# SobeyMIL/MVOC

Hardware: AMD Instinct MI355X
Metric: UNet3D denoising steps/sec, 16x512^2 frames, inversion+compose (higher is better)
Workload: dtype f16

## Files before the change

include/mvoc_hip.h:

```cpp
#ifndef MVOC_HIP_H
#define MVOC_HIP_H

#include <stddef.h>
#include <stdint.h>

#ifdef __cplusplus
extern "C" {
#endif

#define MVOC_VERSION 100

int mvoc_version(void);
const char* mvoc_last_error(void);

enum { MVOC_A_PLAIN = 0, MVOC_A_CONV3X3 = 1, MVOC_A_TEMPORAL3 = 2 };
enum { MVOC_ACT_NONE = 0, MVOC_ACT_GEGLU = 1, MVOC_ACT_SILU = 2, MVOC_ACT_GELU = 3 };

typedef struct mvoc_gemm_desc {
  const void* a;
  const void* a2;
  const void* w;
  void* out;
  const void* bias;
  const void* rowadd;
  const void* resid;
  int64_t m, n, k;
  int32_t n_store;
  int32_t ldo, ldr, ld_rowadd, rowadd_div;
  int32_t a_mode;
  int32_t lda, lda2;
  int32_t c1;
  int32_t cin;
  int32_t nimg, hout, wout, hsrc, wsrc, stride, upsample, hup, wup;
  int32_t frames, hw;
  int32_t act;
  int32_t tile;
  int32_t split_k;
  void* workspace;
  size_t workspace_bytes;
  const void* ln_rowsum;
  const void* ln_bias;
  float ln_eps;
  int32_t pad_mode;
  const void* ln_stats;
  void* chan_sums;
  void* row_moments;
// ... 196 lines not shown
```

mvoc_amd/_ffi.py:

```python
import ctypes as C
import os

import torch

_HERE = os.path.dirname(os.path.abspath(__file__))
LIB_PATH = os.environ.get("MVOC_HIP_LIB") or os.path.join(_HERE, "libmvoc_hip.so")

ABI_VERSION = 100

A_PLAIN, A_CONV3X3, A_TEMPORAL3 = 0, 1, 2
ACT_NONE, ACT_GEGLU, ACT_SILU, ACT_GELU = 0, 1, 2, 3
FAMILIES = ("gemm", "flash_attn", "temporal_attn", "groupnorm", "layernorm", "pnp", "misc", "temporal_fused")

vp, i32, i64, f32, f64, sz = C.c_void_p, C.c_int32, C.c_int64, C.c_float, C.c_double, C.c_size_t


class GemmDesc(C.Structure):
    _fields_ = [("a", vp), ("a2", vp), ("w", vp), ("out", vp), ("bias", vp), ("rowadd", vp), ("resid", vp),
                ("m", i64), ("n", i64), ("k", i64), ("n_store", i32), ("ldo", i32), ("ldr", i32), ("ld_rowadd", i32),
                ("rowadd_div", i32), ("a_mode", i32), ("lda", i32), ("lda2", i32), ("c1", i32), ("cin", i32),
                ("nimg", i32), ("hout", i32), ("wout", i32), ("hsrc", i32), ("wsrc", i32), ("stride", i32),
                ("upsample", i32), ("hup", i32), ("wup", i32), ("frames", i32), ("hw", i32), ("act", i32), ("tile", i32),
                ("split_k", i32), ("workspace", vp), ("workspace_bytes", sz), ("ln_rowsum", vp), ("ln_bias", vp),
                ("ln_eps", f32), ("pad_mode", i32), ("ln_stats", vp), ("chan_sums", vp), ("row_moments", vp),
# ... 11 lines not shown
class TAttnDesc(C.Structure):
    _fields_ = [("q", vp), ("k", vp), ("v", vp), ("out", vp),
                ("q_bs", i64), ("q_ps", i64), ("q_ts", i64), ("k_bs", i64), ("k_ps", i64), ("k_ts", i64),
                ("v_bs", i64), ("v_ps", i64), ("v_ts", i64), ("o_bs", i64), ("o_ps", i64), ("o_ts", i64),
                ("nsample", i32), ("hw", i32), ("heads", i32), ("frames", i32)]


class GnDesc(C.Structure):
    _fields_ = [("x", vp), ("x2", vp), ("gamma", vp), ("beta", vp), ("out", vp), ("workspace", vp),
                ("workspace_bytes", sz), ("nsample", i32), ("rows_per_sample", i32), ("c", i32), ("c1", i32),
                ("groups", i32), ("silu", i32), ("eps", f32), ("chan_sums", vp), ("chan_sums2", vp)]


class TFusedDesc(C.Structure):
    _fields_ = [("x", vp), ("wp", vp), ("ln_rowsum", vp), ("ln_bias", vp), ("out", vp), ("nsample", i32), ("frames", i32),
                ("hw", i32), ("c", i32), ("heads", i32), ("ln_eps", f32)]


class XsDesc(C.Structure):
    _fields_ = [("x", vp), ("wp", vp), ("resid", vp), ("out", vp), ("m", i64),
                ("n", i32), ("k", i32), ("n_store", i32), ("ldo", i32), ("ldr", i32), ("act", i32), ("normalize", i32),
                ("ln_eps", C.c_float), ("wp_set_rows", i64)]


class PnpDesc(C.Structure):
    _fields_ = [("x", vp), ("x2", vp), ("masks", vp), ("chunk_stride", i64), ("f_stride", i64), ("p_stride", i64),
                ("nobj", i32), ("frames", i32), ("height", i32), ("width", i32), ("channels", i32), ("mask_h", i32),
                ("mask_w", i32), ("base_chunk0", i32), ("ndst", i32)]


SIGNATURES = {
    "mvoc_version": (i32, []),
    "mvoc_last_error": (C.c_char_p, []),
    "mvoc_gemm_f16": (i32, [C.POINTER(GemmDesc), vp]),
    "mvoc_gemm_workspace_bytes": (sz, [i64, i64, i64]),
    "mvoc_gemm_chan_sums_written": (i32, []),
    "mvoc_gemm_row_moments_written": (i32, []),
    "mvoc_row_stats_from_moments_f32": (i32, [vp, i64, i32, i32, i32, f32, vp, vp]),
    "mvoc_flash_attn_f16": (i32, [C.POINTER(AttnDesc), vp]),
    "mvoc_temporal_attn_f16": (i32, [C.POINTER(TAttnDesc), vp]),
    "mvoc_temporal_qkv_attn_f16": (i32, [C.POINTER(TFusedDesc), vp]),
    "mvoc_xs_linear_f16": (i32, [C.POINTER(XsDesc), vp]),
    "mvoc_groupnorm_workspace_bytes": (sz, [i32, i32, i32, i32]),
    "mvoc_groupnorm_f16": (i32, [C.POINTER(GnDesc), vp]),
    "mvoc_groupnorm_fold_xs_f16": (i32, [C.POINTER(GnDesc), vp, vp, i32, i32, vp, vp]),
    "mvoc_groupnorm_moments_f16": (i32, [C.POINTER(GnDesc), vp, vp]),
    "mvoc_groupnorm_apply_moments_f16": (i32, [C.POINTER(GnDesc), vp, i32, vp]),
    "mvoc_layernorm_f16": (i32, [vp, vp, vp, vp, i64, i32, f32, vp]),
    "mvoc_row_stats_f16": (i32, [vp, vp, i64, i32, f32, vp]),
    "mvoc_pnp_blend_scatter_tokens": (i32, [C.POINTER(PnpDesc), vp]),
    "mvoc_pnp_blend_scatter_nchw": (i32, [C.POINTER(PnpDesc), vp]),
    "mvoc_pnp_blend_scatter_tokens_mapped": (i32, [C.POINTER(PnpDesc), i32, C.POINTER(i32), vp]),
    "mvoc_pnp_blend_scatter_nchw_mapped": (i32, [C.POINTER(PnpDesc), i32, C.POINTER(i32), vp]),
    "mvoc_pnp_blend_scatter_tokens_variants": (i32, [C.POINTER(PnpDesc), i32, C.POINTER(i32), i32, vp]),
    "mvoc_pnp_blend_scatter_nchw_variants": (i32, [C.POINTER(PnpDesc), i32, C.POINTER(i32), i32, vp]),
    "mvoc_pnp_blend_scatter_tokens_variants_sel": (i32, [C.POINTER(PnpDesc), i32, C.POINTER(i32), i32, C.c_uint32, vp]),
    "mvoc_pnp_blend_scatter_nchw_variants_sel": (i32, [C.POINTER(PnpDesc), i32, C.POINTER(i32), i32, C.c_uint32, vp]),
    "mvoc_pnp_blend_scatter_tokens_placed": (i32, [C.POINTER(PnpDesc), i32, C.POINTER(i32), i32, C.c_uint32, vp, vp]),
    "mvoc_pnp_blend_scatter_nchw_placed": (i32, [C.POINTER(PnpDesc), i32, C.POINTER(i32), i32, C.c_uint32, vp, vp]),
    "mvoc_pnp_blend_scatter_tokens_placed_variants": (i32, [C.POINTER(PnpDesc), i32, C.POINTER(i32), i32, C.c_uint32, vp, vp]),
    "mvoc_pnp_blend_scatter_nchw_placed_variants": (i32, [C.POINTER(PnpDesc), i32, C.POINTER(i32), i32, C.c_uint32, vp, vp]),
    "mvoc_shift_planes_f16": (i32, [vp, vp, i32, i32, i32, i32, vp, vp]),
    "mvoc_pnp_blend_scatter_tokens_resampled": (i32, [C.POINTER(PnpDesc), i32, C.POINTER(i32), i32, C.c_uint32, vp, vp]),
    "mvoc_pnp_blend_scatter_nchw_resampled": (i32, [C.POINTER(PnpDesc), i32, C.POINTER(i32), i32, C.c_uint32, vp, vp]),
    "mvoc_pnp_blend_scatter_tokens_resampled_variants": (i32, [C.POINTER(PnpDesc), i32, C.POINTER(i32), i32, C.c_uint32, vp, vp]),
    "mvoc_pnp_blend_scatter_nchw_resampled_variants": (i32, [C.POINTER(PnpDesc), i32, C.POINTER(i32), i32, C.c_uint32, vp, vp]),
# ... 71 lines not shown
```

mvoc_amd/csrc/runtime.hip:

```cpp
#include <stdarg.h>

#include <mutex>
#include <vector>

#include "common.h"

namespace {
thread_local char g_err[512] = "";

struct ProfRec {
  hipEvent_t e0, e1;
  int fam;
  double work;
};
std::mutex g_prof_mu;
bool g_prof_on = false;
std::vector<ProfRec*> g_prof_recs;
}

void mvoc_set_error(const char* fmt, ...) {
  va_list ap;
  va_start(ap, fmt);
  vsnprintf(g_err, sizeof(g_err), fmt, ap);
  va_end(ap);
}

int mvoc_check_launch(const char* what) {
  hipError_t e = hipGetLastError();
  if (e != hipSuccess) {
    mvoc_set_error("%s: %s", what, hipGetErrorString(e));
    return -3;
  }
  return 0;
}

MvocProfScope::MvocProfScope(int fam_, hipStream_t s, double work) : fam(fam_), stream(s), rec(nullptr) {
  if (!g_prof_on) return;
  ProfRec* r = new ProfRec;
  r->fam = fam_;
  r->work = work;
  if (hipEventCreate(&r->e0) != hipSuccess || hipEventCreate(&r->e1) != hipSuccess) {
    delete r;
    return;
  }
  (void)hipEventRecord(r->e0, s);
  rec = r;
}

MvocProfScope::~MvocProfScope() {
  if (!rec) return;
  ProfRec* r = (ProfRec*)rec;
  (void)hipEventRecord(r->e1, stream);
  std::lock_guard<std::mutex> lk(g_prof_mu);
  g_prof_recs.push_back(r);
}

extern "C" int mvoc_version(void) { return MVOC_VERSION; }
extern "C" const char* mvoc_last_error(void) { return g_err; }

extern "C" int mvoc_prof_enable(int on) {
  g_prof_on = on != 0;
  return 0;
}

extern "C" int mvoc_prof_reset(void) {
  std::lock_guard<std::mutex> lk(g_prof_mu);
  for (ProfRec* r : g_prof_recs) {
    (void)hipEventDestroy(r->e0);
    (void)hipEventDestroy(r->e1);
    delete r;
  }
  g_prof_recs.clear();
  return 0;
}

extern "C" int mvoc_prof_collect(double* ms, int64_t* launches, double* work) {
  std::lock_guard<std::mutex> lk(g_prof_mu);
  for (int i = 0; i < MVOC_FAM_COUNT; ++i) {
    if (ms) ms[i] = 0;
    if (launches) launches[i] = 0;
    if (work) work[i] = 0;
  }
  for (ProfRec* r : g_prof_recs) {
    float t = 0;
    if (hipEventElapsedTime(&t, r->e0, r->e1) != hipSuccess) {
      mvoc_set_error("prof_collect: event not complete (synchronise the stream first)");
      return -3;
    }
    if (ms) ms[r->fam] += t;
// ... 6 lines not shown
```

mvoc_amd/csrc/xslin.hip:

```cpp
#include <stdlib.h>

#include "common.h"

namespace {

struct XsArgs {
  const half_t* x;
  const half_t* wp;
  const half_t* resid;
  half_t* out;
  long M;
  int N, n_store, ldo, ldr, act, normalize;
  float eps;
  unsigned long long* stamps;
  int lab;
  long set_rows;
  long set_bytes;
};

#ifdef MVOC_PP_LAB
#define XS_STAMP(t) asm volatile("s_memtime %0\n\ts_waitcnt lgkmcnt(0)" : "=s"(t)::"memory")
#define XS_ACC(slot, a, b) (acc_t[slot] += (b) - (a))
#else
#define XS_STAMP(t) do { } while (0)
#define XS_ACC(slot, a, b) do { } while (0)
#endif

template <int N_>
__device__ __forceinline__ void xs_wait() {
  asm volatile("s_waitcnt vmcnt(%0)" ::"n"(N_) : "memory");
}
__device__ __forceinline__ void xs_wait_n(int n) {
  switch (n) {
    case 0: xs_wait<0>(); break;   case 1: xs_wait<1>(); break;   case 2: xs_wait<2>(); break;   case 3: xs_wait<3>(); break;
    case 4: xs_wait<4>(); break;   case 5: xs_wait<5>(); break;   case 6: xs_wait<6>(); break;   case 7: xs_wait<7>(); break;
    case 8: xs_wait<8>(); break;   case 9: xs_wait<9>(); break;   case 10: xs_wait<10>(); break; case 11: xs_wait<11>(); break;
    case 12: xs_wait<12>(); break; case 13: xs_wait<13>(); break; case 14: xs_wait<14>(); break; case 15: xs_wait<15>(); break;
    case 16: xs_wait<16>(); break; case 17: xs_wait<17>(); break; case 18: xs_wait<18>(); break; case 19: xs_wait<19>(); break;
    case 20: xs_wait<20>(); break; case 21: xs_wait<21>(); break; default: xs_wait<22>(); break;
  }
}

template <int NK, int RG, int ACT>
__global__ __launch_bounds__(256, 2) void xslin_kernel(const XsArgs p) {
  constexpr int NS = 3, NW = 4;
  constexpr int NP = NK + 1;
  constexpr int STAGE = NP * 1024;
  constexpr int K = NK * 16;
  constexpr int RBUF = 4096;
  __shared__ __attribute__((aligned(1024))) char smem[NS * STAGE + NW * RBUF];
  const int tid = threadIdx.x, lane = tid & 63;
  const int wave = __builtin_amdgcn_readfirstlane(tid >> 6);
  const int r = lane & 31, h = lane >> 5;
  long ms[RG];
#pragma unroll
  for (int g = 0; g < RG; ++g) {
    const long m = (long)blockIdx.x * (NW * 32 * RG) + wave * (32 * RG) + 32 * g + r;
    ms[g] = m < p.M ? m : p.M - 1;
  }

  const char* wp_set = reinterpret_cast<const char*>(p.wp) +
                       (p.set_rows > 0 ? ((long)blockIdx.x * (NW * 32 * RG) / p.set_rows) * p.set_bytes : 0);
  const int pw = (NP - wave + NW - 1) / NW;
  const int T = p.N / 32;
  auto issue = [&](int st) {
    const char* src = wp_set + (size_t)st * STAGE + lane * 16;
    char* dst = smem + (st % NS) * STAGE;
#pragma unroll
    for (int i = 0; i < (NP + NW - 1) / NW; ++i) {
      const int j = wave + NW * i;
      if (j < NP)
        __builtin_amdgcn_global_load_lds((const __attribute__((address_space(1))) void*)(src + j * 1024),
                                         (__attribute__((address_space(3))) void*)(dst + j * 1024), 16, 0, 0);
    }
  };
  char* resbuf = smem + NS * STAGE + wave * RBUF;
  auto res_slot = [&](int tile, int g, int j) -> char* {
    return resbuf + (RG == 1 ? (tile & 1) * 2048 : g * 2048) + j * 1024;
  };
  auto issue_resid = [&](int tile) {
#pragma unroll
    for (int g = 0; g < RG; ++g)
#pragma unroll
      for (int j = 0; j < 2; ++j) {
        int n = 32 * tile + 16 * j + 8 * h;
        n = n < p.n_store ? n : p.n_store - 8;
        __builtin_amdgcn_global_load_lds((const __attribute__((address_space(1))) void*)(p.resid + ms[g] * p.ldr + n),
                                         (__attribute__((address_space(3))) void*)res_slot(tile, g, j), 16, 0, 0);
      }
  };
  const int S = 2 * RG, R = p.resid ? 2 * RG : 0;
  constexpr bool GEGLU = ACT == MVOC_ACT_GEGLU;
  constexpr bool geglu = GEGLU;
  constexpr int PW_LO = NP / NW, PW_HI = (NP + NW - 1) / NW;
  auto wait_stage = [&](int st) {
    if (st >= 2 && st + 1 < T) {
      if (geglu) {
        if (pw == PW_HI) xs_wait<PW_HI + 2 * RG>(); else xs_wait<PW_LO + 2 * RG>();
      } else if (p.resid) {
        if (pw == PW_HI) xs_wait<PW_HI + 8 * RG>(); else xs_wait<PW_LO + 8 * RG>();
      } else {
        if (pw == PW_HI) xs_wait<PW_HI + 4 * RG>(); else xs_wait<PW_LO + 4 * RG>();
      }
      return;
    }
    const int dma_next = st + 1 < T ? pw : 0;
    int n;
    if (st == 0) n = dma_next;
    else if (geglu) n = dma_next + (st >= 2 ? S : 0);
    else n = dma_next + (st >= 2 ? 2 * (R + S) : R + S);
    xs_wait_n(n);
  };
  auto wait_resid = [&](int st) {
    if (RG == 1) xs_wait_n((st >= 1 ? S : 0) + (st + 2 < T ? pw : 0) + (st + 1 < T ? R : 0));
    else xs_wait_n(st >= 1 && st + 2 < T ? pw : 0);
  };

  half8_t xf[RG][NK];
#pragma unroll
  for (int g = 0; g < RG; ++g) {
    const half_t* xr = p.x + ms[g] * K + 8 * h;
#pragma unroll
    for (int s = 0; s < NK; ++s) xf[g][s] = *reinterpret_cast<const half8_t*>(xr + 16 * s);
  }
  if (p.resid) issue_resid(0);
  for (int st = 0; st < NS - 1 && st < T; ++st) issue(st);
  if (p.normalize) {
    const half2_t one2 = {(half_t)1.0f, (half_t)1.0f};
#pragma unroll
    for (int g = 0; g < RG; ++g) {
      float s1 = 0.f;
#pragma unroll
      for (int s = 0; s < NK; ++s)
#pragma unroll
        for (int e = 0; e < 4; ++e) {
          const half2_t v2 = {xf[g][s][2 * e], xf[g][s][2 * e + 1]};
          s1 = __builtin_amdgcn_fdot2(v2, one2, s1, false);
        }
      s1 += __shfl_xor(s1, 32);
      const float mu = s1 / (float)K;
      const half_t c16 = (half_t)mu;
      const half2_t c2 = {c16, c16};
      float t1 = 0.f, t2 = 0.f;
#pragma unroll
      for (int s = 0; s < NK; ++s)
#pragma unroll
        for (int e = 0; e < 4; ++e) {
          const half2_t v2 = {xf[g][s][2 * e], xf[g][s][2 * e + 1]};
          const half2_t d2 = v2 - c2;
          t1 = __builtin_amdgcn_fdot2(d2, one2, t1, false);
          t2 = __builtin_amdgcn_fdot2(d2, d2, t2, false);
        }
      t1 += __shfl_xor(t1, 32);
      t2 += __shfl_xor(t2, 32);
      const float dm = t1 / (float)K;
      const float rs = rsqrtf(fmaxf(t2 / (float)K - dm * dm, 0.f) + p.eps);
#pragma unroll
      for (int s = 0; s < NK; ++s)
#pragma unroll
        for (int e = 0; e < 8; ++e) xf[g][s][e] = (half_t)(((float)xf[g][s][e] - mu) * rs);
    }
  }

  int stage = 0;
  constexpr int PD = NK < 8 ? NK : (RG == 1 ? 8 : (GEGLU ? 2 : 4));
  const char* cslot = smem;
#ifdef MVOC_PP_LAB
  unsigned long long acc_t[6] = {0, 0, 0, 0, 0, 0}, ta = 0, tb = 0, tc = 0, td = 0, te = 0, tstart = 0;
  XS_STAMP(tstart);
  te = tstart;
#endif
  auto run_stage = [&](f32x16 (&acc)[RG]) {
    XS_STAMP(ta);
    XS_ACC(3, te, ta);
    wait_stage(stage);
    XS_STAMP(tb);
    XS_ACC(0, ta, tb);
    __builtin_amdgcn_sched_barrier(0);
    __builtin_amdgcn_s_barrier();
    __builtin_amdgcn_sched_barrier(0);
    XS_STAMP(tc);
    XS_ACC(1, tb, tc);
    if (stage + NS - 1 < T) issue(stage + NS - 1);
    if (RG == 1 && p.resid && stage + 1 < T) issue_resid(stage + 1);
    cslot = smem + (stage % NS) * STAGE;
    const char* wl = cslot + lane * 16;
    half8_t wf[PD];
#pragma unroll
    for (int i = 0; i < PD; ++i) wf[i] = *reinterpret_cast<const half8_t*>(wl + i * 1024);
    __builtin_amdgcn_sched_group_barrier(0x100, PD, 0);
#pragma unroll
    for (int s = 0; s < NK; ++s) {
#pragma unroll
      for (int g = 0; g < RG; ++g) acc[g] = __builtin_amdgcn_mfma_f32_32x32x16_f16(wf[s % PD], xf[g][s], acc[g], 0, 0, 0);
      if (s + PD < NK) wf[s % PD] = *reinterpret_cast<const half8_t*>(wl + (s + PD) * 1024);
      __builtin_amdgcn_sched_group_barrier(0x008, RG, 0);
      __builtin_amdgcn_sched_group_barrier(0x100, 1, 0);
    }
#ifdef MVOC_PP_LAB
    asm volatile("s_nop 0" ::"v"(acc[0][0]), "v"(acc[RG - 1][15]));
#endif
    XS_STAMP(te);
    XS_ACC(2, tc, te);
    ++stage;
  };
  auto cvec4 = [&](const char* slot, int c) -> f32x4 { return *reinterpret_cast<const f32x4*>(slot + NK * 1024 + c * 4); };
  auto store_tile = [&](unsigned (&pk)[4][2], int nout, int tile, int g) {
#pragma unroll
    for (int qq = 0; qq < 4; qq += 2)
#pragma unroll
      for (int w2 = 0; w2 < 2; ++w2) {
        const auto sw = __builtin_amdgcn_permlane32_swap(pk[qq][w2], pk[qq + 1][w2], false, false);
        pk[qq][w2] = sw[0];
        pk[qq + 1][w2] = sw[1];
      }
#pragma unroll
    for (int j = 0; j < 2; ++j) {
      const int n = nout + 16 * j + 8 * h;
      uint4 v = {pk[2 * j][0], pk[2 * j][1], pk[2 * j + 1][0], pk[2 * j + 1][1]};
      if (p.resid) {
        half8_t a = __builtin_bit_cast(half8_t, v);
        const half8_t b = *reinterpret_cast<const half8_t*>(res_slot(tile, g, j) + lane * 16);
#pragma unroll
        for (int e = 0; e < 8; ++e) a[e] = (half_t)((float)a[e] + (float)b[e]);
        v = __builtin_bit_cast(uint4, a);
      }
      if (n >= p.n_store) continue;
#ifdef MVOC_PP_LAB
      if (p.lab & 1) { asm volatile("" ::"v"(v.x), "v"(v.y), "v"(v.z), "v"(v.w)); continue; }
      if (p.lab & 2) {
        *reinterpret_cast<uint4*>(p.out + ((long)blockIdx.x * 1024 + (wave * 2 * RG + 2 * g + j)) * 512 + lane * 8 + (long)(nout / 32) * 0) = v;
        continue;
      }
#endif
      *reinterpret_cast<uint4*>(p.out + ms[g] * p.ldo + n) = v;
    }
  };

  if constexpr (GEGLU) {
    for (int t = 0; t + 1 < T; t += 2) {
      f32x16 acc[RG];
#pragma unroll
      for (int g = 0; g < RG; ++g)
#pragma unroll
        for (int e = 0; e < 16; ++e) acc[g][e] = 0.f;
      run_stage(acc);
      half2_t hv[RG][8];
#pragma unroll
      for (int q = 0; q < 4; ++q) {
        const f32x4 cvl = cvec4(cslot, 8 * q + 4 * h);
#pragma unroll
        for (int g = 0; g < RG; ++g) {
          hv[g][2 * q] = half2_t{(half_t)(acc[g][4 * q] + cvl[0]), (half_t)(acc[g][4 * q + 1] + cvl[1])};
          hv[g][2 * q + 1] = half2_t{(half_t)(acc[g][4 * q + 2] + cvl[2]), (half_t)(acc[g][4 * q + 3] + cvl[3])};
        }
      }
#pragma unroll
      for (int g = 0; g < RG; ++g)
#pragma unroll
        for (int e = 0; e < 16; ++e) acc[g][e] = 0.f;
      run_stage(acc);
#pragma unroll
      for (int g = 0; g < RG; ++g) {
        unsigned pk[4][2];
#pragma unroll
        for (int q = 0; q < 4; ++q) {
          const f32x4 cgt = cvec4(cslot, 8 * q + 4 * h);
          half_t o[4];
#pragma unroll
          for (int e = 0; e < 4; ++e) {
            const float gv = r16(acc[g][4 * q + e] + cgt[e]);
            o[e] = (half_t)((float)hv[g][2 * q + (e >> 1)][e & 1] * r16(gelu_fast_f(gv)));
          }
          const half2_t lo = {o[0], o[1]}, hi = {o[2], o[3]};
          pk[q][0] = __builtin_bit_cast(unsigned, lo);
          pk[q][1] = __builtin_bit_cast(unsigned, hi);
        }
        store_tile(pk, 16 * t, t + 1, g);
      }
    }
  } else {
    for (int t = 0; t < T; ++t) {
      f32x16 acc[RG];
#pragma unroll
      for (int g = 0; g < RG; ++g)
#pragma unroll
        for (int e = 0; e < 16; ++e) acc[g][e] = 0.f;
      run_stage(acc);
      if (p.resid) wait_resid(t);
#pragma unroll
      for (int g = 0; g < RG; ++g) {
        unsigned pk[4][2];
#pragma unroll
        for (int q = 0; q < 4; ++q) {
          const f32x4 cv = cvec4(cslot, 8 * q + 4 * h);
          half_t o[4];
#pragma unroll
          for (int e = 0; e < 4; ++e) {
            float v = r16(acc[g][4 * q + e] + cv[e]);
            if constexpr (ACT == MVOC_ACT_SILU) v = r16(silu_f(v));
            else if constexpr (ACT == MVOC_ACT_GELU) v = r16(gelu_fast_f(v));
            o[e] = (half_t)v;
          }
          const half2_t lo = {o[0], o[1]}, hi = {o[2], o[3]};
          pk[q][0] = __builtin_bit_cast(unsigned, lo);
          pk[q][1] = __builtin_bit_cast(unsigned, hi);
        }
        store_tile(pk, 32 * t, t, g);
      }
      if (RG == 2 && p.resid && t + 1 < T) {
        asm volatile("s_waitcnt lgkmcnt(0)" ::: "memory");
        issue_resid(t + 1);
      }
    }
  }
#ifdef MVOC_PP_LAB
  XS_STAMP(ta);
  XS_ACC(3, te, ta);
  if (p.stamps && blockIdx.x == 0 && wave == 0 && lane == 0) {
    for (int i = 0; i < 4; ++i) p.stamps[i] = acc_t[i];
    p.stamps[4] = ta - tstart;
    p.stamps[5] = (unsigned long long)T;
  }
#endif
}

}

extern "C" int mvoc_xs_linear_f16(const mvoc_xs_desc* d, void* stream) {
  MVOC_REQUIRE(d && d->x && d->wp && d->out, -1, "xs_linear: null operand");
  MVOC_REQUIRE(d->m > 0 && d->n > 0 && d->n % 32 == 0, -1, "xs_linear: m > 0, n %% 32 == 0");
  MVOC_REQUIRE(d->act >= MVOC_ACT_NONE && d->act <= MVOC_ACT_GELU, -1, "xs_linear: bad act %d", d->act);
  MVOC_REQUIRE(!(d->resid && d->act == MVOC_ACT_GEGLU), -2, "xs_linear: no residual with GEGLU");
  MVOC_REQUIRE(d->k == 64 || d->k == 128 || d->k == 320, -2, "xs_linear: k (%d) must be 64, 128 or 320", d->k);
  MVOC_REQUIRE(d->act != MVOC_ACT_GEGLU || d->n % 64 == 0, -2, "xs_linear: GEGLU needs n %% 64 == 0");
  const int ns = d->n_store > 0 ? d->n_store : (d->act == MVOC_ACT_GEGLU ? d->n / 2 : d->n);
  MVOC_REQUIRE(ns > (d->act == MVOC_ACT_GEGLU ? d->n / 2 : d->n) - 32, -2, "xs_linear: n_store may only trim the last 32-channel tile");
  MVOC_REQUIRE(ns % 8 == 0 && d->ldo % 8 == 0 && ((uintptr_t)d->out & 15) == 0 &&
                   (d->resid == nullptr || (d->ldr % 8 == 0 && ((uintptr_t)d->resid & 15) == 0)),
               -2, "xs_linear: outputs / residual must be 16-byte addressable per 8 channels");
  MVOC_REQUIRE(((uintptr_t)d->x & 15) == 0 && ((uintptr_t)d->wp & 15) == 0, -2,
               "xs_linear: x / wp must be 16-byte addressable (both are read in 16-byte pieces)");
  XsArgs a;
  a.x = (const half_t*)d->x; a.wp = (const half_t*)d->wp;
  a.resid = (const half_t*)d->resid; a.out = (half_t*)d->out;
  a.M = d->m; a.N = d->n; a.n_store = ns; a.ldo = d->ldo; a.ldr = d->ldr; a.act = d->act; a.normalize = d->normalize; a.eps = d->ln_eps;
  static const int force_rg = getenv("MVOC_XS_RG") ? atoi(getenv("MVOC_XS_RG")) : 0;
  const int rg = force_rg ? force_rg : (d->m >= 131072 && d->k == 320 ? 2 : 1);
  a.stamps = nullptr;
  a.lab = 0;
  a.set_rows = d->wp_set_rows;
  a.set_bytes = (long)(d->n / 32) * (d->k / 16 + 1) * 1024;
  MVOC_REQUIRE(d->wp_set_rows >= 0 && (d->wp_set_rows == 0 || (d->wp_set_rows % (128 * rg) == 0 && d->m % d->wp_set_rows == 0)), -2,
               "xs_linear: wp_set_rows (%ld) must be a multiple of the %d rows of a block and divide m", (long)d->wp_set_rows, 128 * rg);
#ifdef MVOC_PP_LAB
  if (const char* e = getenv("MVOC_XS_STAMPS")) a.stamps = (unsigned long long*)strtoull(e, nullptr, 10);
  a.lab = getenv("MVOC_XS_LAB") ? atoi(getenv("MVOC_XS_LAB")) : 0;
#endif
  const long nblk = (d->m + 128 * rg - 1) / (128 * rg);
  MVOC_REQUIRE(nblk < 0x7fffffffL, -2, "xs_linear: grid too large");
  hipStream_t s = (hipStream_t)stream;
  MvocProfScope prof(MVOC_FAM_GEMM, s, 2.0 * (double)d->m * d->n * d->k);
  const dim3 grid((unsigned)nblk), blk(256);
#define XS_LAUNCH(NK_, RG_)                                                                                        \
  do {                                                                                                             \
    if (d->act == MVOC_ACT_GEGLU) hipLaunchKernelGGL((xslin_kernel<NK_, RG_, MVOC_ACT_GEGLU>), grid, blk, 0, s, a);  \
    else if (d->act == MVOC_ACT_SILU) hipLaunchKernelGGL((xslin_kernel<NK_, RG_, MVOC_ACT_SILU>), grid, blk, 0, s, a); \
    else if (d->act == MVOC_ACT_GELU) hipLaunchKernelGGL((xslin_kernel<NK_, RG_, MVOC_ACT_GELU>), grid, blk, 0, s, a); \
    else hipLaunchKernelGGL((xslin_kernel<NK_, RG_, MVOC_ACT_NONE>), grid, blk, 0, s, a);                          \
  } while (0)
  if (d->k == 320 && rg == 2) XS_LAUNCH(20, 2);
  else if (d->k == 320) XS_LAUNCH(20, 1);
  else if (d->k == 128 && rg == 2) XS_LAUNCH(8, 2);
  else if (d->k == 128) XS_LAUNCH(8, 1);
  else if (rg == 2) XS_LAUNCH(4, 2);
  else XS_LAUNCH(4, 1);
#undef XS_LAUNCH
  return mvoc_check_launch("xslin_kernel");
}
```

Measured before the change: 24.25.

## Add 16x16x32 MFMA variant of xs_linear kernel, default for k=320 none/GEGLU

Moves the xs_linear kernel body into a shared header and builds it twice: the original 32x32x16 MFMA path and a new path using 16x16x32 f16 MFMAs. The new path remaps the weight-fragment layout in shared memory, the accumulator layout, the bias indexing, the LayerNorm lane reductions and the output permute (permlane16 swaps). It is selected by default for k=320 with no activation or GEGLU, and an environment switch can override the choice. The aim is higher MFMA throughput or better scheduling on CDNA for the common k=320 projections, at the cost of more reductions and shuffles and a second compiled kernel variant.

New measurement: 24.32 (median of 6 runs). About the same (+0.3%).

```diff
diff --git a/include/mvoc_hip.h b/include/mvoc_hip.h
--- a/include/mvoc_hip.h
+++ b/include/mvoc_hip.h
@@ -12,6 +12,9 @@
 
 int mvoc_version(void);
 const char* mvoc_last_error(void);
+
+enum { MVOC_MFMA16_XS = 0, MVOC_MFMA16_COUNT = 1 };
+int mvoc_mfma16_switch(int family);
 
 enum { MVOC_A_PLAIN = 0, MVOC_A_CONV3X3 = 1, MVOC_A_TEMPORAL3 = 2 };
 enum { MVOC_ACT_NONE = 0, MVOC_ACT_GEGLU = 1, MVOC_ACT_SILU = 2, MVOC_ACT_GELU = 3 };
diff --git a/mvoc_amd/_ffi.py b/mvoc_amd/_ffi.py
--- a/mvoc_amd/_ffi.py
+++ b/mvoc_amd/_ffi.py
@@ -67,6 +67,7 @@
 SIGNATURES = {
     "mvoc_version": (i32, []),
     "mvoc_last_error": (C.c_char_p, []),
+    "mvoc_mfma16_switch": (i32, [i32]),
     "mvoc_gemm_f16": (i32, [C.POINTER(GemmDesc), vp]),
     "mvoc_gemm_workspace_bytes": (sz, [i64, i64, i64]),
     "mvoc_gemm_chan_sums_written": (i32, []),
diff --git a/mvoc_amd/csrc/runtime.hip b/mvoc_amd/csrc/runtime.hip
--- a/mvoc_amd/csrc/runtime.hip
+++ b/mvoc_amd/csrc/runtime.hip
@@ -1,4 +1,5 @@
 #include <stdarg.h>
+#include <stdlib.h>
 
 #include <mutex>
 #include <vector>
@@ -55,6 +56,19 @@
   g_prof_recs.push_back(r);
 }
 
+namespace {
+int env_switch(const char* name) {
+  const char* e = getenv(name);
+  if (!e || !e[0]) return -1;
+  if ((e[0] == '0' || e[0] == '1') && !e[1]) return e[0] - '0';
+  fprintf(stderr, "libmvoc_hip: %s=%s ignored (0 or 1)\n", name, e);
+  return -1;
+}
+const int g_mfma16[MVOC_MFMA16_COUNT] = {env_switch("MVOC_MFMA16_XS")};
+}
+
+extern "C" int mvoc_mfma16_switch(int family) { return family >= 0 && family < MVOC_MFMA16_COUNT ? g_mfma16[family] : -2; }
+
 extern "C" int mvoc_version(void) { return MVOC_VERSION; }
 extern "C" const char* mvoc_last_error(void) { return g_err; }
 
diff --git a/mvoc_amd/csrc/xslin.hip b/mvoc_amd/csrc/xslin.hip
--- a/mvoc_amd/csrc/xslin.hip
+++ b/mvoc_amd/csrc/xslin.hip
@@ -1,4 +1,6 @@
 #include <stdlib.h>
+
+#include <type_traits>
 
 #include "common.h"
 
@@ -41,291 +43,20 @@
   }
 }
 
-template <int NK, int RG, int ACT>
-__global__ __launch_bounds__(256, 2) void xslin_kernel(const XsArgs p) {
-  constexpr int NS = 3, NW = 4;
-  constexpr int NP = NK + 1;
-  constexpr int STAGE = NP * 1024;
-  constexpr int K = NK * 16;
-  constexpr int RBUF = 4096;
-  __shared__ __attribute__((aligned(1024))) char smem[NS * STAGE + NW * RBUF];
-  const int tid = threadIdx.x, lane = tid & 63;
-  const int wave = __builtin_amdgcn_readfirstlane(tid >> 6);
-  const int r = lane & 31, h = lane >> 5;
-  long ms[RG];
-#pragma unroll
-  for (int g = 0; g < RG; ++g) {
-    const long m = (long)blockIdx.x * (NW * 32 * RG) + wave * (32 * RG) + 32 * g + r;
-    ms[g] = m < p.M ? m : p.M - 1;
-  }
+#define XS_KERNEL xslin_kernel
+#define XS_MF16 false
+#include "xslin_body.h"
+#undef XS_KERNEL
+#undef XS_MF16
+#define XS_KERNEL xslin16_kernel
+#define XS_MF16 true
+#include "xslin_body.h"
+#undef XS_KERNEL
+#undef XS_MF16
 
-  const char* wp_set = reinterpret_cast<const char*>(p.wp) +
-                       (p.set_rows > 0 ? ((long)blockIdx.x * (NW * 32 * RG) / p.set_rows) * p.set_bytes : 0);
-  const int pw = (NP - wave + NW - 1) / NW;
-  const int T = p.N / 32;
-  auto issue = [&](int st) {
-    const char* src = wp_set + (size_t)st * STAGE + lane * 16;
-    char* dst = smem + (st % NS) * STAGE;
-#pragma unroll
-    for (int i = 0; i < (NP + NW - 1) / NW; ++i) {
-      const int j = wave + NW * i;
-      if (j < NP)
-        __builtin_amdgcn_global_load_lds((const __attribute__((address_space(1))) void*)(src + j * 1024),
-                                         (__attribute__((address_space(3))) void*)(dst + j * 1024), 16, 0, 0);
-    }
-  };
-  char* resbuf = smem + NS * STAGE + wave * RBUF;
-  auto res_slot = [&](int tile, int g, int j) -> char* {
-    return resbuf + (RG == 1 ? (tile & 1) * 2048 : g * 2048) + j * 1024;
-  };
-  auto issue_resid = [&](int tile) {
-#pragma unroll
-    for (int g = 0; g < RG; ++g)
-#pragma unroll
-      for (int j = 0; j < 2; ++j) {
-        int n = 32 * tile + 16 * j + 8 * h;
-        n = n < p.n_store ? n : p.n_store - 8;
-        __builtin_amdgcn_global_load_lds((const __attribute__((address_space(1))) void*)(p.resid + ms[g] * p.ldr + n),
-                                         (__attribute__((address_space(3))) void*)res_slot(tile, g, j), 16, 0, 0);
-      }
-  };
-  const int S = 2 * RG, R = p.resid ? 2 * RG : 0;
-  constexpr bool GEGLU = ACT == MVOC_ACT_GEGLU;
-  constexpr bool geglu = GEGLU;
-  constexpr int PW_LO = NP / NW, PW_HI = (NP + NW - 1) / NW;
-  auto wait_stage = [&](int st) {
-    if (st >= 2 && st + 1 < T) {
-      if (geglu) {
-        if (pw == PW_HI) xs_wait<PW_HI + 2 * RG>(); else xs_wait<PW_LO + 2 * RG>();
-      } else if (p.resid) {
-        if (pw == PW_HI) xs_wait<PW_HI + 8 * RG>(); else xs_wait<PW_LO + 8 * RG>();
-      } else {
-        if (pw == PW_HI) xs_wait<PW_HI + 4 * RG>(); else xs_wait<PW_LO + 4 * RG>();
-      }
-      return;
-    }
-    const int dma_next = st + 1 < T ? pw : 0;
-    int n;
-    if (st == 0) n = dma_next;
-    else if (geglu) n = dma_next + (st >= 2 ? S : 0);
-    else n = dma_next + (st >= 2 ? 2 * (R + S) : R + S);
-    xs_wait_n(n);
-  };
-  auto wait_resid = [&](int st) {
-    if (RG == 1) xs_wait_n((st >= 1 ? S : 0) + (st + 2 < T ? pw : 0) + (st + 1 < T ? R : 0));
-    else xs_wait_n(st >= 1 && st + 2 < T ? pw : 0);
-  };
-
-  half8_t xf[RG][NK];
-#pragma unroll
-  for (int g = 0; g < RG; ++g) {
-    const half_t* xr = p.x + ms[g] * K + 8 * h;
-#pragma unroll
-    for (int s = 0; s < NK; ++s) xf[g][s] = *reinterpret_cast<const half8_t*>(xr + 16 * s);
-  }
-  if (p.resid) issue_resid(0);
-  for (int st = 0; st < NS - 1 && st < T; ++st) issue(st);
-  if (p.normalize) {
-    const half2_t one2 = {(half_t)1.0f, (half_t)1.0f};
-#pragma unroll
-    for (int g = 0; g < RG; ++g) {
-      float s1 = 0.f;
-#pragma unroll
-      for (int s = 0; s < NK; ++s)
-#pragma unroll
-        for (int e = 0; e < 4; ++e) {
-          const half2_t v2 = {xf[g][s][2 * e], xf[g][s][2 * e + 1]};
-          s1 = __builtin_amdgcn_fdot2(v2, one2, s1, false);
-        }
-      s1 += __shfl_xor(s1, 32);
-      const float mu = s1 / (float)K;
-      const half_t c16 = (half_t)mu;
-      const half2_t c2 = {c16, c16};
-      float t1 = 0.f, t2 = 0.f;
-#pragma unroll
-      for (int s = 0; s < NK; ++s)
-#pragma unroll
-        for (int e = 0; e < 4; ++e) {
-          const half2_t v2 = {xf[g][s][2 * e], xf[g][s][2 * e + 1]};
-          const half2_t d2 = v2 - c2;
-          t1 = __builtin_amdgcn_fdot2(d2, one2, t1, false);
-          t2 = __builtin_amdgcn_fdot2(d2, d2, t2, false);
-        }
-      t1 += __shfl_xor(t1, 32);
-      t2 += __shfl_xor(t2, 32);
-      const float dm = t1 / (float)K;
-      const float rs = rsqrtf(fmaxf(t2 / (float)K - dm * dm, 0.f) + p.eps);
-#pragma unroll
-      for (int s = 0; s < NK; ++s)
-#pragma unroll
-        for (int e = 0; e < 8; ++e) xf[g][s][e] = (half_t)(((float)xf[g][s][e] - mu) * rs);
-    }
-  }
-
-  int stage = 0;
-  constexpr int PD = NK < 8 ? NK : (RG == 1 ? 8 : (GEGLU ? 2 : 4));
-  const char* cslot = smem;
-#ifdef MVOC_PP_LAB
-  unsigned long long acc_t[6] = {0, 0, 0, 0, 0, 0}, ta = 0, tb = 0, tc = 0, td = 0, te = 0, tstart = 0;
-  XS_STAMP(tstart);
-  te = tstart;
-#endif
-  auto run_stage = [&](f32x16 (&acc)[RG]) {
-    XS_STAMP(ta);
-    XS_ACC(3, te, ta);
-    wait_stage(stage);
-    XS_STAMP(tb);
-    XS_ACC(0, ta, tb);
-    __builtin_amdgcn_sched_barrier(0);
-    __builtin_amdgcn_s_barrier();
-    __builtin_amdgcn_sched_barrier(0);
-    XS_STAMP(tc);
-    XS_ACC(1, tb, tc);
-    if (stage + NS - 1 < T) issue(stage + NS - 1);
-    if (RG == 1 && p.resid && stage + 1 < T) issue_resid(stage + 1);
-    cslot = smem + (stage % NS) * STAGE;
-    const char* wl = cslot + lane * 16;
-    half8_t wf[PD];
-#pragma unroll
-    for (int i = 0; i < PD; ++i) wf[i] = *reinterpret_cast<const half8_t*>(wl + i * 1024);
-    __builtin_amdgcn_sched_group_barrier(0x100, PD, 0);
-#pragma unroll
-    for (int s = 0; s < NK; ++s) {
-#pragma unroll
-      for (int g = 0; g < RG; ++g) acc[g] = __builtin_amdgcn_mfma_f32_32x32x16_f16(wf[s % PD], xf[g][s], acc[g], 0, 0, 0);
-      if (s + PD < NK) wf[s % PD] = *reinterpret_cast<const half8_t*>(wl + (s + PD) * 1024);
-      __builtin_amdgcn_sched_group_barrier(0x008, RG, 0);
-      __builtin_amdgcn_sched_group_barrier(0x100, 1, 0);
-    }
-#ifdef MVOC_PP_LAB
-    asm volatile("s_nop 0" ::"v"(acc[0][0]), "v"(acc[RG - 1][15]));
-#endif
-    XS_STAMP(te);
-    XS_ACC(2, tc, te);
-    ++stage;
-  };
-  auto cvec4 = [&](const char* slot, int c) -> f32x4 { return *reinterpret_cast<const f32x4*>(slot + NK * 1024 + c * 4); };
-  auto store_tile = [&](unsigned (&pk)[4][2], int nout, int tile, int g) {
-#pragma unroll
-    for (int qq = 0; qq < 4; qq += 2)
-#pragma unroll
-      for (int w2 = 0; w2 < 2; ++w2) {
-        const auto sw = __builtin_amdgcn_permlane32_swap(pk[qq][w2], pk[qq + 1][w2], false, false);
-        pk[qq][w2] = sw[0];
-        pk[qq + 1][w2] = sw[1];
-      }
-#pragma unroll
-    for (int j = 0; j < 2; ++j) {
-      const int n = nout + 16 * j + 8 * h;
-      uint4 v = {pk[2 * j][0], pk[2 * j][1], pk[2 * j + 1][0], pk[2 * j + 1][1]};
-      if (p.resid) {
-        half8_t a = __builtin_bit_cast(half8_t, v);
-        const half8_t b = *reinterpret_cast<const half8_t*>(res_slot(tile, g, j) + lane * 16);
-#pragma unroll
-        for (int e = 0; e < 8; ++e) a[e] = (half_t)((float)a[e] + (float)b[e]);
-        v = __builtin_bit_cast(uint4, a);
-      }
-      if (n >= p.n_store) continue;
-#ifdef MVOC_PP_LAB
-      if (p.lab & 1) { asm volatile("" ::"v"(v.x), "v"(v.y), "v"(v.z), "v"(v.w)); continue; }
-      if (p.lab & 2) {
-        *reinterpret_cast<uint4*>(p.out + ((long)blockIdx.x * 1024 + (wave * 2 * RG + 2 * g + j)) * 512 + lane * 8 + (long)(nout / 32) * 0) = v;
-        continue;
-      }
-#endif
-      *reinterpret_cast<uint4*>(p.out + ms[g] * p.ldo + n) = v;
-    }
-  };
-
-  if constexpr (GEGLU) {
-    for (int t = 0; t + 1 < T; t += 2) {
-      f32x16 acc[RG];
-#pragma unroll
-      for (int g = 0; g < RG; ++g)
-#pragma unroll
-        for (int e = 0; e < 16; ++e) acc[g][e] = 0.f;
-      run_stage(acc);
-      half2_t hv[RG][8];
-#pragma unroll
-      for (int q = 0; q < 4; ++q) {
-        const f32x4 cvl = cvec4(cslot, 8 * q + 4 * h);
-#pragma unroll
-        for (int g = 0; g < RG; ++g) {
-          hv[g][2 * q] = half2_t{(half_t)(acc[g][4 * q] + cvl[0]), (half_t)(acc[g][4 * q + 1] + cvl[1])};
-          hv[g][2 * q + 1] = half2_t{(half_t)(acc[g][4 * q + 2] + cvl[2]), (half_t)(acc[g][4 * q + 3] + cvl[3])};
-        }
-      }
-#pragma unroll
-      for (int g = 0; g < RG; ++g)
-#pragma unroll
-        for (int e = 0; e < 16; ++e) acc[g][e] = 0.f;
-      run_stage(acc);
-#pragma unroll
-      for (int g = 0; g < RG; ++g) {
-        unsigned pk[4][2];
-#pragma unroll
-        for (int q = 0; q < 4; ++q) {
-          const f32x4 cgt = cvec4(cslot, 8 * q + 4 * h);
-          half_t o[4];
-#pragma unroll
-          for (int e = 0; e < 4; ++e) {
-            const float gv = r16(acc[g][4 * q + e] + cgt[e]);
-            o[e] = (half_t)((float)hv[g][2 * q + (e >> 1)][e & 1] * r16(gelu_fast_f(gv)));
-          }
-          const half2_t lo = {o[0], o[1]}, hi = {o[2], o[3]};
-          pk[q][0] = __builtin_bit_cast(unsigned, lo);
-          pk[q][1] = __builtin_bit_cast(unsigned, hi);
-        }
-        store_tile(pk, 16 * t, t + 1, g);
-      }
-    }
-  } else {
-    for (int t = 0; t < T; ++t) {
-      f32x16 acc[RG];
-#pragma unroll
-      for (int g = 0; g < RG; ++g)
-#pragma unroll
-        for (int e = 0; e < 16; ++e) acc[g][e] = 0.f;
-      run_stage(acc);
-      if (p.resid) wait_resid(t);
-#pragma unroll
-      for (int g = 0; g < RG; ++g) {
-        unsigned pk[4][2];
-#pragma unroll
-        for (int q = 0; q < 4; ++q) {
-          const f32x4 cv = cvec4(cslot, 8 * q + 4 * h);
-          half_t o[4];
-#pragma unroll
-          for (int e = 0; e < 4; ++e) {
-            float v = r16(acc[g][4 * q + e] + cv[e]);
-            if constexpr (ACT == MVOC_ACT_SILU) v = r16(silu_f(v));
-            else if constexpr (ACT == MVOC_ACT_GELU) v = r16(gelu_fast_f(v));
-            o[e] = (half_t)v;
-          }
-          const half2_t lo = {o[0], o[1]}, hi = {o[2], o[3]};
-          pk[q][0] = __builtin_bit_cast(unsigned, lo);
-          pk[q][1] = __builtin_bit_cast(unsigned, hi);
-        }
-        store_tile(pk, 32 * t, t, g);
-      }
-      if (RG == 2 && p.resid && t + 1 < T) {
-        asm volatile("s_waitcnt lgkmcnt(0)" ::: "memory");
-        issue_resid(t + 1);
-      }
-    }
-  }
-#ifdef MVOC_PP_LAB
-  XS_STAMP(ta);
-  XS_ACC(3, te, ta);
-  if (p.stamps && blockIdx.x == 0 && wave == 0 && lane == 0) {
-    for (int i = 0; i < 4; ++i) p.stamps[i] = acc_t[i];
-    p.stamps[4] = ta - tstart;
-    p.stamps[5] = (unsigned long long)T;
-  }
-#endif
 }
 
-}
+#define XS_MF16_DEFAULT(k, act) ((k) == 320 && ((act) == MVOC_ACT_NONE || (act) == MVOC_ACT_GEGLU))
 
 extern "C" int mvoc_xs_linear_f16(const mvoc_xs_desc* d, void* stream) {
   MVOC_REQUIRE(d && d->x && d->wp && d->out, -1, "xs_linear: null operand");
@@ -362,12 +93,19 @@
   hipStream_t s = (hipStream_t)stream;
   MvocProfScope prof(MVOC_FAM_GEMM, s, 2.0 * (double)d->m * d->n * d->k);
   const dim3 grid((unsigned)nblk), blk(256);
-#define XS_LAUNCH(NK_, RG_)                                                                                        \
-  do {                                                                                                             \
-    if (d->act == MVOC_ACT_GEGLU) hipLaunchKernelGGL((xslin_kernel<NK_, RG_, MVOC_ACT_GEGLU>), grid, blk, 0, s, a);  \
-    else if (d->act == MVOC_ACT_SILU) hipLaunchKernelGGL((xslin_kernel<NK_, RG_, MVOC_ACT_SILU>), grid, blk, 0, s, a); \
-    else if (d->act == MVOC_ACT_GELU) hipLaunchKernelGGL((xslin_kernel<NK_, RG_, MVOC_ACT_GELU>), grid, blk, 0, s, a); \
-    else hipLaunchKernelGGL((xslin_kernel<NK_, RG_, MVOC_ACT_NONE>), grid, blk, 0, s, a);                          \
+  const int mf16_env = mvoc_mfma16_switch(MVOC_MFMA16_XS);
+  const bool mf16 = mf16_env >= 0 ? mf16_env != 0 : XS_MF16_DEFAULT(d->k, d->act);
+#define XS_LAUNCH_ACT(KERNEL_, NK_, RG_)                                                                        \
+  do {                                                                                                            \
+    if (d->act == MVOC_ACT_GEGLU) hipLaunchKernelGGL((KERNEL_<NK_, RG_, MVOC_ACT_GEGLU>), grid, blk, 0, s, a);     \
+    else if (d->act == MVOC_ACT_SILU) hipLaunchKernelGGL((KERNEL_<NK_, RG_, MVOC_ACT_SILU>), grid, blk, 0, s, a);  \
+    else if (d->act == MVOC_ACT_GELU) hipLaunchKernelGGL((KERNEL_<NK_, RG_, MVOC_ACT_GELU>), grid, blk, 0, s, a);  \
+    else hipLaunchKernelGGL((KERNEL_<NK_, RG_, MVOC_ACT_NONE>), grid, blk, 0, s, a);                              \
+  } while (0)
+#define XS_LAUNCH(NK_, RG_)                            \
+  do {                                                 \
+    if (mf16) XS_LAUNCH_ACT(xslin16_kernel, NK_, RG_); \
+    else XS_LAUNCH_ACT(xslin_kernel, NK_, RG_);        \
   } while (0)
   if (d->k == 320 && rg == 2) XS_LAUNCH(20, 2);
   else if (d->k == 320) XS_LAUNCH(20, 1);
@@ -376,5 +114,6 @@
   else if (rg == 2) XS_LAUNCH(4, 2);
   else XS_LAUNCH(4, 1);
 #undef XS_LAUNCH
+#undef XS_LAUNCH_ACT
   return mvoc_check_launch("xslin_kernel");
 }
diff --git a/mvoc_amd/csrc/xslin_body.h b/mvoc_amd/csrc/xslin_body.h
--- /dev/null
+++ b/mvoc_amd/csrc/xslin_body.h
@@ -0,0 +1,355 @@
+template <int NK, int RG, int ACT>
+__global__ __launch_bounds__(256, 2) void XS_KERNEL(const XsArgs p) {
+  constexpr bool MF16 = XS_MF16 && NK > 0;
+  static_assert(NK % 2 == 0, "a K-32 step is two pieces");
+  constexpr int NS = 3, NW = 4;
+  constexpr int NP = NK + 1;
+  constexpr int STAGE = NP * 1024;
+  constexpr int K = NK * 16;
+  constexpr int RBUF = 4096;
+  __shared__ __attribute__((aligned(1024))) char smem[NS * STAGE + NW * RBUF];
+  const int tid = threadIdx.x, lane = tid & 63;
+  const int wave = __builtin_amdgcn_readfirstlane(tid >> 6);
+  const int r = lane & 31, h = lane >> 5;
+  const int kq = lane >> 4;
+  long ms[RG];
+#pragma unroll
+  for (int g = 0; g < RG; ++g) {
+    const long m = (long)blockIdx.x * (NW * 32 * RG) + wave * (32 * RG) + 32 * g + r;
+    ms[g] = m < p.M ? m : p.M - 1;
+  }
+
+  const char* wp_set = reinterpret_cast<const char*>(p.wp) +
+                       (p.set_rows > 0 ? ((long)blockIdx.x * (NW * 32 * RG) / p.set_rows) * p.set_bytes : 0);
+  const int pw = (NP - wave + NW - 1) / NW;
+  const int T = p.N / 32;
+  auto issue = [&](int st) {
+    const char* src = wp_set + (size_t)st * STAGE + lane * 16;
+    char* dst = smem + (st % NS) * STAGE;
+#pragma unroll
+    for (int i = 0; i < (NP + NW - 1) / NW; ++i) {
+      const int j = wave + NW * i;
+      if (j < NP)
+        __builtin_amdgcn_global_load_lds((const __attribute__((address_space(1))) void*)(src + j * 1024),
+                                         (__attribute__((address_space(3))) void*)(dst + j * 1024), 16, 0, 0);
+    }
+  };
+  char* resbuf = smem + NS * STAGE + wave * RBUF;
+  auto res_slot = [&](int tile, int g, int j) -> char* {
+    return resbuf + (RG == 1 ? (tile & 1) * 2048 : g * 2048) + j * 1024;
+  };
+  auto issue_resid = [&](int tile) {
+#pragma unroll
+    for (int g = 0; g < RG; ++g)
+#pragma unroll
+      for (int j = 0; j < 2; ++j) {
+        int n = 32 * tile + 16 * j + 8 * h;
+        n = n < p.n_store ? n : p.n_store - 8;
+        __builtin_amdgcn_global_load_lds((const __attribute__((address_space(1))) void*)(p.resid + ms[g] * p.ldr + n),
+                                         (__attribute__((address_space(3))) void*)res_slot(tile, g, j), 16, 0, 0);
+      }
+  };
+  const int S = 2 * RG, R = p.resid ? 2 * RG : 0;
+  constexpr bool GEGLU = ACT == MVOC_ACT_GEGLU;
+  constexpr bool geglu = GEGLU;
+  constexpr int PW_LO = NP / NW, PW_HI = (NP + NW - 1) / NW;
+  auto wait_stage = [&](int st) {
+    if (st >= 2 && st + 1 < T) {
+      if (geglu) {
+        if (pw == PW_HI) xs_wait<PW_HI + 2 * RG>(); else xs_wait<PW_LO + 2 * RG>();
+      } else if (p.resid) {
+        if (pw == PW_HI) xs_wait<PW_HI + 8 * RG>(); else xs_wait<PW_LO + 8 * RG>();
+      } else {
+        if (pw == PW_HI) xs_wait<PW_HI + 4 * RG>(); else xs_wait<PW_LO + 4 * RG>();
+      }
+      return;
+    }
+    const int dma_next = st + 1 < T ? pw : 0;
+    int n;
+    if (st == 0) n = dma_next;
+    else if (geglu) n = dma_next + (st >= 2 ? S : 0);
+    else n = dma_next + (st >= 2 ? 2 * (R + S) : R + S);
+    xs_wait_n(n);
+  };
+  auto wait_resid = [&](int st) {
+    if (RG == 1) xs_wait_n((st >= 1 ? S : 0) + (st + 2 < T ? pw : 0) + (st + 1 < T ? R : 0));
+    else xs_wait_n(st >= 1 && st + 2 < T ? pw : 0);
+  };
+
+  constexpr int NR = MF16 ? 2 : 1;
+  half8_t xf[RG][NK];
+#pragma unroll
+  for (int g = 0; g < RG; ++g) {
+    if constexpr (MF16) {
+#pragma unroll
+      for (int rb = 0; rb < 2; ++rb) {
+        const long m = (long)blockIdx.x * (NW * 32 * RG) + wave * (32 * RG) + 32 * g + 16 * rb + (lane & 15);
+        const half_t* xr = p.x + (m < p.M ? m : p.M - 1) * K + 8 * kq;
+#pragma unroll
+        for (int s = 0; s < NK / 2; ++s) xf[g][2 * s + rb] = *reinterpret_cast<const half8_t*>(xr + 32 * s);
+      }
+    } else {
+      const half_t* xr = p.x + ms[g] * K + 8 * h;
+#pragma unroll
+      for (int s = 0; s < NK; ++s) xf[g][s] = *reinterpret_cast<const half8_t*>(xr + 16 * s);
+    }
+  }
+  if (p.resid) issue_resid(0);
+  for (int st = 0; st < NS - 1 && st < T; ++st) issue(st);
+  if (p.normalize) {
+    const half2_t one2 = {(half_t)1.0f, (half_t)1.0f};
+#pragma unroll
+    for (int g = 0; g < RG; ++g)
+#pragma unroll
+    for (int rr = 0; rr < NR; ++rr) {
+      float s1 = 0.f;
+#pragma unroll
+      for (int s = rr; s < NK; s += NR)
+#pragma unroll
+        for (int e = 0; e < 4; ++e) {
+          const half2_t v2 = {xf[g][s][2 * e], xf[g][s][2 * e + 1]};
+          s1 = __builtin_amdgcn_fdot2(v2, one2, s1, false);
+        }
+      s1 += __shfl_xor(s1, 32);
+      if constexpr (MF16) s1 += __shfl_xor(s1, 16);
+      const float mu = s1 / (float)K;
+      const half_t c16 = (half_t)mu;
+      const half2_t c2 = {c16, c16};
+      float t1 = 0.f, t2 = 0.f;
+#pragma unroll
+      for (int s = rr; s < NK; s += NR)
+#pragma unroll
+        for (int e = 0; e < 4; ++e) {
+          const half2_t v2 = {xf[g][s][2 * e], xf[g][s][2 * e + 1]};
+          const half2_t d2 = v2 - c2;
+          t1 = __builtin_amdgcn_fdot2(d2, one2, t1, false);
+          t2 = __builtin_amdgcn_fdot2(d2, d2, t2, false);
+        }
+      t1 += __shfl_xor(t1, 32);
+      t2 += __shfl_xor(t2, 32);
+      if constexpr (MF16) {
+        t1 += __shfl_xor(t1, 16);
+        t2 += __shfl_xor(t2, 16);
+      }
+      const float dm = t1 / (float)K;
+      const float rs = rsqrtf(fmaxf(t2 / (float)K - dm * dm, 0.f) + p.eps);
+#pragma unroll
+      for (int s = rr; s < NK; s += NR)
+#pragma unroll
+        for (int e = 0; e < 8; ++e) xf[g][s][e] = (half_t)(((float)xf[g][s][e] - mu) * rs);
+    }
+  }
+
+  using acc_t = typename std::conditional<MF16, f32x4[4], f32x16>::type;
+  auto acc_at = [](const acc_t& a, int q, int e) -> float {
+    if constexpr (MF16) return a[q][e];
+    else return a[4 * q + e];
+  };
+  auto acc_zero = [](f32x4 (&acc)[RG][4]) {
+#pragma unroll
+    for (int g = 0; g < RG; ++g)
+#pragma unroll
+      for (int q = 0; q < 4; ++q)
+#pragma unroll
+        for (int e = 0; e < 4; ++e) acc[g][q][e] = 0.f;
+  };
+  auto cq = [&](int q) -> int { return MF16 ? 16 * (q >> 1) + 4 * kq : 8 * q + 4 * h; };
+  int stage = 0;
+  constexpr int PD = NK < 8 ? NK : (RG == 1 ? 8 : (GEGLU ? 2 : 4));
+  const char* cslot = smem;
+#ifdef MVOC_PP_LAB
+  unsigned long long acc_t[6] = {0, 0, 0, 0, 0, 0}, ta = 0, tb = 0, tc = 0, td = 0, te = 0, tstart = 0;
+  XS_STAMP(tstart);
+  te = tstart;
+#endif
+  auto run_stage = [&](acc_t (&acc)[RG]) {
+    XS_STAMP(ta);
+    XS_ACC(3, te, ta);
+    wait_stage(stage);
+    XS_STAMP(tb);
+    XS_ACC(0, ta, tb);
+    __builtin_amdgcn_sched_barrier(0);
+    __builtin_amdgcn_s_barrier();
+    __builtin_amdgcn_sched_barrier(0);
+    XS_STAMP(tc);
+    XS_ACC(1, tb, tc);
+    if (stage + NS - 1 < T) issue(stage + NS - 1);
+    if (RG == 1 && p.resid && stage + 1 < T) issue_resid(stage + 1);
+    cslot = smem + (stage % NS) * STAGE;
+    const char* wl = cslot + (MF16 ? (kq >> 1) * 1024 + ((lane & 15) + 32 * (kq & 1)) * 16 : lane * 16);
+    auto frag = [&](int s) -> half8_t { return *reinterpret_cast<const half8_t*>(wl + (MF16 ? (s >> 1) * 2048 + (s & 1) * 256 : s * 1024)); };
+    half8_t wf[PD];
+#pragma unroll
+    for (int i = 0; i < PD; ++i) wf[i] = frag(i);
+    __builtin_amdgcn_sched_group_barrier(0x100, PD, 0);
+#pragma unroll
+    for (int s = 0; s < NK; ++s) {
+#pragma unroll
+      for (int g = 0; g < RG; ++g) {
+        if constexpr (MF16) {
+#pragma unroll
+          for (int rb = 0; rb < 2; ++rb)
+            acc[g][2 * (s & 1) + rb] = __builtin_amdgcn_mfma_f32_16x16x32_f16(wf[s % PD], xf[g][(s & ~1) + rb], acc[g][2 * (s & 1) + rb], 0, 0, 0);
+        } else {
+          acc[g] = __builtin_amdgcn_mfma_f32_32x32x16_f16(wf[s % PD], xf[g][s], acc[g], 0, 0, 0);
+        }
+      }
+      if (s + PD < NK) wf[s % PD] = frag(s + PD);
+      __builtin_amdgcn_sched_group_barrier(0x008, NR * RG, 0);
+      __builtin_amdgcn_sched_group_barrier(0x100, 1, 0);
+    }
+#ifdef MVOC_PP_LAB
+    asm volatile("s_nop 0" ::"v"(acc_at(acc[0], 0, 0)), "v"(acc_at(acc[RG - 1], 3, 3)));
+#endif
+    XS_STAMP(te);
+    XS_ACC(2, tc, te);
+    ++stage;
+  };
+  auto cvec4 = [&](const char* slot, int c) -> f32x4 { return *reinterpret_cast<const f32x4*>(slot + NK * 1024 + c * 4); };
+  auto store_tile = [&](unsigned (&pk)[4][2], int nout, int tile, int g) {
+#pragma unroll
+    for (int qq = 0; qq < 4; qq += 2)
+#pragma unroll
+      for (int w2 = 0; w2 < 2; ++w2) {
+        if constexpr (MF16) {
+          const auto sw = __builtin_amdgcn_permlane16_swap(pk[qq][w2], pk[qq + 1][w2], false, false);
+          pk[qq][w2] = sw[0];
+          pk[qq + 1][w2] = sw[1];
+        } else {
+          const auto sw = __builtin_amdgcn_permlane32_swap(pk[qq][w2], pk[qq + 1][w2], false, false);
+          pk[qq][w2] = sw[0];
+          pk[qq + 1][w2] = sw[1];
+        }
+      }
+#pragma unroll
+    for (int j = 0; j < 2; ++j) {
+      const int n = nout + 16 * j + 8 * h;
+      uint4 v = {pk[2 * j][0], pk[2 * j][1], pk[2 * j + 1][0], pk[2 * j + 1][1]};
+      if (p.resid) {
+        half8_t a = __builtin_bit_cast(half8_t, v);
+        const half8_t b = *reinterpret_cast<const half8_t*>(res_slot(tile, g, j) + lane * 16);
+#pragma unroll
+        for (int e = 0; e < 8; ++e) a[e] = (half_t)((float)a[e] + (float)b[e]);
+        v = __builtin_bit_cast(uint4, a);
+      }
+      if (n >= p.n_store) continue;
+#ifdef MVOC_PP_LAB
+      if (p.lab & 1) { asm volatile("" ::"v"(v.x), "v"(v.y), "v"(v.z), "v"(v.w)); continue; }
+      if (p.lab & 2) {
+        *reinterpret_cast<uint4*>(p.out + ((long)blockIdx.x * 1024 + (wave * 2 * RG + 2 * g + j)) * 512 + lane * 8 + (long)(nout / 32) * 0) = v;
+        continue;
+      }
+#endif
+      *reinterpret_cast<uint4*>(p.out + ms[g] * p.ldo + n) = v;
+    }
+  };
+
+  if constexpr (GEGLU) {
+    for (int t = 0; t + 1 < T; t += 2) {
+      acc_t acc[RG];
+      if constexpr (MF16) {
+        acc_zero(acc);
+      } else {
+#pragma unroll
+        for (int g = 0; g < RG; ++g)
+#pragma unroll
+          for (int e = 0; e < 16; ++e) acc[g][e] = 0.f;
+      }
+      run_stage(acc);
+      half2_t hv[RG][8];
+#pragma unroll
+      for (int q = 0; q < 4; ++q) {
+        const f32x4 cvl = cvec4(cslot, cq(q));
+#pragma unroll
+        for (int g = 0; g < RG; ++g) {
+          hv[g][2 * q] = half2_t{(half_t)(acc_at(acc[g], q, 0) + cvl[0]), (half_t)(acc_at(acc[g], q, 1) + cvl[1])};
+          hv[g][2 * q + 1] = half2_t{(half_t)(acc_at(acc[g], q, 2) + cvl[2]), (half_t)(acc_at(acc[g], q, 3) + cvl[3])};
+        }
+      }
+      if constexpr (MF16) {
+#pragma unroll
+        for (int g = 0; g < RG; ++g)
+#pragma unroll
+          for (int i = 0; i < 8; ++i) {
+            unsigned u = __builtin_bit_cast(unsigned, hv[g][i]);
+            asm volatile("" : "+v"(u));
+            hv[g][i] = __builtin_bit_cast(half2_t, u);
+          }
+      }
+      if constexpr (MF16) {
+        acc_zero(acc);
+      } else {
+#pragma unroll
+        for (int g = 0; g < RG; ++g)
+#pragma unroll
+          for (int e = 0; e < 16; ++e) acc[g][e] = 0.f;
+      }
+      run_stage(acc);
+#pragma unroll
+      for (int g = 0; g < RG; ++g) {
+        unsigned pk[4][2];
+#pragma unroll
+        for (int q = 0; q < 4; ++q) {
+          const f32x4 cgt = cvec4(cslot, cq(q));
+          half_t o[4];
+#pragma unroll
+          for (int e = 0; e < 4; ++e) {
+            const float gv = r16(acc_at(acc[g], q, e) + cgt[e]);
+            o[e] = (half_t)((float)hv[g][2 * q + (e >> 1)][e & 1] * r16(gelu_fast_f(gv)));
+          }
+          const half2_t lo = {o[0], o[1]}, hi = {o[2], o[3]};
+          pk[q][0] = __builtin_bit_cast(unsigned, lo);
+          pk[q][1] = __builtin_bit_cast(unsigned, hi);
+        }
+        store_tile(pk, 16 * t, t + 1, g);
+      }
+    }
+  } else {
+    for (int t = 0; t < T; ++t) {
+      acc_t acc[RG];
+      if constexpr (MF16) {
+        acc_zero(acc);
+      } else {
+#pragma unroll
+        for (int g = 0; g < RG; ++g)
+#pragma unroll
+          for (int e = 0; e < 16; ++e) acc[g][e] = 0.f;
+      }
+      run_stage(acc);
+      if (p.resid) wait_resid(t);
+#pragma unroll
+      for (int g = 0; g < RG; ++g) {
+        unsigned pk[4][2];
+#pragma unroll
+        for (int q = 0; q < 4; ++q) {
+          const f32x4 cv = cvec4(cslot, cq(q));
+          half_t o[4];
+#pragma unroll
+          for (int e = 0; e < 4; ++e) {
+            float v = r16(acc_at(acc[g], q, e) + cv[e]);
+            if constexpr (ACT == MVOC_ACT_SILU) v = r16(silu_f(v));
+            else if constexpr (ACT == MVOC_ACT_GELU) v = r16(gelu_fast_f(v));
+            o[e] = (half_t)v;
+          }
+          const half2_t lo = {o[0], o[1]}, hi = {o[2], o[3]};
+          pk[q][0] = __builtin_bit_cast(unsigned, lo);
+          pk[q][1] = __builtin_bit_cast(unsigned, hi);
+        }
+        store_tile(pk, 32 * t, t, g);
+      }
+      if (RG == 2 && p.resid && t + 1 < T) {
+        asm volatile("s_waitcnt lgkmcnt(0)" ::: "memory");
+        issue_resid(t + 1);
+      }
+    }
+  }
+#ifdef MVOC_PP_LAB
+  XS_STAMP(ta);
+  XS_ACC(3, te, ta);
+  if (p.stamps && blockIdx.x == 0 && wave == 0 && lane == 0) {
+    for (int i = 0; i < 4; ++i) p.stamps[i] = acc_t[i];
+    p.stamps[4] = ta - tstart;
+    p.stamps[5] = (unsigned long long)T;
+  }
+#endif
+}
```
